# skovaka/UNCALLED

Measured on NVIDIA H100. Metric: reads/sec mapped (E. coli, 4k-sample reads) at 1/2/4/8 H100 vs CPU ref, higher is better.
Workload: dtype f32/f64 events, u32 FM index

## Files before the change

### uncalled_b200/csrc/unc_device.cuh

```cuda
#pragma once
#include "unc_warp.cuh"

typedef uint8_t u8;
typedef uint16_t u16;
typedef uint32_t u32;
typedef int32_t i32;
typedef uint64_t u64;

#define UNC_NKMER 1024
#define UNC_KMASK 0x3FFu
#define UNC_SEED_LEN 22u
#define UNC_NGEN 24u
#define UNC_PATH_MASK 0x3FFFFFu
#define UNC_PATH_TAIL 0x200000u
#define UNC_INVALID 0x80000000u
#define UNC_BLK 32u


struct DevIndex {
    const uint4 *bwt;
    const u32 *sa;
    const u32 *sa_full;
    const uint2 *kmer_range;
    const float *lv_mean, *lv_var2, *lognorm;
    const float *thresh;
    u32 primary, seq_len;
    u32 L2[5];
    u32 start_bits;
    const uint4 *occ2;
    const struct K2V2Tab *kt;
};

#define K2V2_MAX_MERGED 64u
struct alignas(16) K2V2Tab {
    u16 kslot[UNC_NKMER];
    u16 gkmer[UNC_NKMER];
    u16 gmeta[UNC_NKMER];
    u16 mk[K2V2_MAX_MERGED];
    u8 ksub[UNC_NKMER];
};

UNC_DEV u32 unc_L2(const DevIndex &ix, u32 c) {
    return c == 0 ? ix.L2[0] : c == 1 ? ix.L2[1] : c == 2 ? ix.L2[2] : c == 3 ? ix.L2[3] : ix.L2[4];
}

struct DevParams {
    u32 max_rep_copy, max_paths, max_consec_stay, max_events, min_rep_len;
    float max_stay_frac, min_seed_prob;
    u32 min_map_len;
    float min_mean_conf, min_top_conf;
    float threshold1, threshold2, peak_height, min_mean, max_mean;
    float bp_per_sec, sample_rate;
    float tgt_mean, tgt_stdv;
};

struct DevReadDesc {
    u64 offset;
    u32 n_samples, dtype;
    float cal_range, cal_offset, cal_digit;
    u32 pad;
};

struct DevRec {
    i32 mapped, fwd, rid, status;
    u32 n_events, events_used, matches, n_clusters;
// ... 598 lines not shown
            blk = de.z; cnt = de.w;
            mm.ren_start = 0; mm.evt_en = 0; mm.ref_st = 0; mm.ren_end = 0; mm.evt_st = 0; mm.total_len = 0;
            if ((u32) lane < cnt) mm = trk_load(t, blk, (u32) lane);
        }
        Clu a;
        a.ren_start = w_shfl(mm.ren_start, (int) mpos); a.evt_en = w_shfl(mm.evt_en, (int) mpos); a.ref_st = w_shfl(mm.ref_st, (int) mpos);
        a.ren_end = w_shfl(mm.ren_end, (int) mpos); a.evt_st = w_shfl(mm.evt_st, (int) mpos); a.total_len = w_shfl(mm.total_len, (int) mpos);
        u32 prev_len = a.total_len;
        clu_update(a, ns);
        if (a.total_len != prev_len) {
            t.len_sum = f_add(t.len_sum, (float) (a.total_len - prev_len));
            lens_replace(t, prev_len, a.total_len);
            if (a.total_len >= p.min_map_len && a.total_len > t.max_map.total_len) t.max_map = a;
        }
        bool in_place = false;
        if (mpos > 0) {
            const u32 ps = w_shfl(mm.ren_start, (int) mpos - 1), pe = w_shfl(mm.evt_en, (int) mpos - 1);
            in_place = clu_less(ps, pe, a.ren_start, a.evt_en);
        } else in_place = md == 0;
        if (in_place) {
            w_sync();
            if (lane == 0) {
                trk_store(t, blk, mpos, a);
                if (mpos == 0) t.dir[md] = make_uint4(a.ren_start, a.evt_en, blk, cnt);
            }
            w_sync();
        } else {
            trk_erase(t, md, mpos);
            trk_insert_unique(t, a);
        }
    } else {
        lens_insert(t, ns.total_len);
        t.len_sum = f_add(t.len_sum, (float) ns.total_len);
        if (ns.total_len >= p.min_map_len && ns.total_len > t.max_map.total_len) t.max_map = ns;
        trk_insert_unique(t, ns, have_lb ? &lb : nullptr);
    }
    PT_TRK(t, 2)
}

UNC_DEV bool trk_get_final(const Tracker &t, const DevParams &p) {
    if (t.max_map.total_len < p.min_map_len || t.n_lens < 2) return false;
    float mean_len = f_div(t.len_sum, (float) t.n_live);
    float second_len = (float) t.top2;
    float sl = (float) t.max_map.total_len;
    return (p.min_mean_conf > 0 && f_div(sl, mean_len) >= p.min_mean_conf) ||
           (p.min_top_conf > 0 && f_div(sl, second_len) >= p.min_top_conf);
}

#define K2_CH_SLOTS 160u
#define K2_V2_DYN_BYTES (16u + K2_MAXSEG * (K2_CH_SLOTS * 8u + K2_CH_SLOTS))
#ifndef K2_MAXSEG
#define K2_MAXSEG 16u
#endif
#define K2_DYN_PER_CHUNK 8u
#define K2_SMEM_BYTES(maxp) (sizeof(K2Shared) + 16 + (size_t) (((maxp) + 31) / 32) * K2_DYN_PER_CHUNK + 32 + K2_V2_DYN_BYTES)
struct K2Tables {
    uint2 kmer_range[UNC_NKMER];
    float thresh[64];
};
struct K2V2 {
    K2V2Tab t;
    u32 kcnt[UNC_NKMER];
    u32 koff[UNC_NKMER];
    u32 kagg[UNC_NKMER];
    u32 fresh_cand[32], fresh_mask[32], fresh_before[32];
    u32 grab;
    u16 mfirst[K2V2_MAX_MERGED];
#if defined(UNC_PHASE_TIMING) && !defined(UNC_EMUL)
    u32 pt_dur[4][K2_MAXSEG];
#endif
};
struct K2Shared {
    K2Tables tb;
    float probs[UNC_NKMER];
    u32 flags[32];
    u32 flags_prev[32];
    u32 sort_hist[256 * K2_MAXSEG];
    uint4 trk_dir[1024];
    u32 *bcnt, *ecnt;
    K2V2 v2;
    unsigned char *v2_stage;
    u32 bc[8];
    u32 n_rows[2];
    u32 verdict[2];
    u32 wk_overflow;
    u32 wl_cnt;
    u32 cnt_blocks, cnt_steps;
    u32 tot_children[2], tot_sources[2];
    DevWork work;
};

#include "unc_pdqsort.cuh"
#ifdef UNC_EMUL
static unsigned long g_emu_tie_stats[2];
#endif
UNC_DEV void write_source(uint4 *rec, uint2 *hist_e, u32 idx, u32 st, u32 en, u32 kmer, float prob) {
    rec[(size_t) idx * 2] = make_uint4(st, en, kmer | (1u << 16), 1u);
    rec[(size_t) idx * 2 + 1] = make_uint4(f2u(prob), f2u(prob), 0u, 0u);
    hist_e[idx] = make_uint2(f2u(prob), 0xFFFFFFFFu);
}

UNC_DEV u32 unc_event_to_bp(u32 evt_i, bool last, float mean_event_len, float bp_per_samp) {
    float v = f_add(f_mul(f_mul((float) evt_i, mean_event_len), bp_per_samp), (float) (last ? 4 : 0));
    return f_to_u32_x86(v);
}

UNC_DEV void unc_k2_cta_setup(const DevIndex &ix, const DevParams &p, K2Shared *sh) {
    const u32 n_slots = (p.max_paths + 31u) >> 5;
    if (c_tid() == 0) {
        char *base = (char *) ((((size_t) (sh + 1)) + 15) & ~(size_t) 15);
        sh->bcnt = (u32 *) base; base += (size_t) n_slots * 4;
        sh->ecnt = (u32 *) base; base += (size_t) n_slots * 4;
        sh->v2_stage = (unsigned char *) ((((size_t) base) + 15) & ~(size_t) 15);
    }
    c_sync();
    for (u32 k = (u32) c_tid(); k < UNC_NKMER; k += (u32) c_nthreads()) {
        sh->tb.kmer_range[k] = ix.kmer_range[k];
    }
    for (u32 k = (u32) c_tid(); k < 64; k += (u32) c_nthreads()) sh->tb.thresh[k] = ix.thresh[k];
    for (u32 k = (u32) c_tid(); k < (u32) (sizeof(K2V2Tab) / 4); k += (u32) c_nthreads()) ((u32 *) &sh->v2.t)[k] = ((const u32 *) ix.kt)[k];
    c_sync();
}

UNC_DEV void unc_k2_write_record(const DevIndex &ix, const DevParams &p, const DevBatch &B, K2Shared *sh, u32 r,
                                 const Tracker &trk, u32 verdict, u32 final_event, u64 n_seeds) {
    const float mel = B.mean_event_len[r];
    const float bp_per_samp = f_div(p.bp_per_sec, p.sample_rate);
    DevRec o;
    o.mapped = 0; o.fwd = 0; o.rid = -1; o.status = verdict == 2u ? -7 : 0;
    o.n_events = B.n_events[r]; o.events_used = final_event; o.matches = 0; o.n_clusters = trk.n_live;
    o.rd_len = f_to_u64(f_mul((float) (u64) B.reads[r].n_samples, bp_per_samp));
    o.rd_st = o.rd_en = o.rf_st = o.rf_en = o.rf_len = 0;
    if (verdict == 1u) {
        const Clu &sc = trk.max_map;
        bool fwd = sc.ref_st < ix.seq_len / 2u;
        u64 sa_st = fwd ? (u64) sc.ref_st : (u64) ix.seq_len - ((u64) sc.ren_end + 4u);
        o.rd_st = unc_event_to_bp(sc.evt_st - UNC_SEED_LEN, false, mel, bp_per_samp);
        o.rd_en = unc_event_to_bp(sc.evt_en, true, mel, bp_per_samp);
        o.rd_len = unc_event_to_bp(final_event, true, mel, bp_per_samp);
        int rid = -1;
        if ((long long) sa_st < (long long) B.l_pac) {
            int left = 0, mid = 0, right = (int) B.n_seqs;
            while (left < right) {
                mid = (left + right) >> 1;
                if (sa_st >= B.seq_offsets[mid]) {
                    if (mid == (int) B.n_seqs - 1) break;
                    if (sa_st < B.seq_offsets[mid + 1]) break;
                    left = mid + 1;
                } else right = mid;
            }
            rid = mid;
        }
        u64 rf_st = 0, rf_len = 0;
        if (rid >= 0) { rf_st = sa_st - B.seq_offsets[rid]; rf_len = B.seq_lens[rid]; }
        o.mapped = 1; o.fwd = fwd ? 1 : 0; o.rid = rid;
        o.rf_st = rf_st; o.rf_len = rf_len;
        o.rf_en = rf_st + ((u64) sc.ren_end - (u64) sc.ref_st + 5u);
        o.matches = (sc.total_len + 4u) & 0xFFFFu;
    }
    o.n_children = ((u64) sh->tot_children[1] << 32) | sh->tot_children[0];
    o.n_sources = ((u64) sh->tot_sources[1] << 32) | sh->tot_sources[0];
    o.n_seeds = n_seeds;
    o.n_occ_blocks = sh->cnt_blocks; o.n_sa_steps = sh->cnt_steps;
    B.out[r] = o;
}

#if defined(UNC_PHASE_TIMING) && !defined(UNC_EMUL)
UNC_DEV long long pt_clock() { long long v; asm volatile("mov.u64 %0, %%clock64;" : "=l"(v) :: "memory"); return v; }
#define PT_DECL unsigned long long pt_acc[32]; for (int _i = 0; _i < 32; _i++) pt_acc[_i] = 0; long long pt_t = pt_clock();
#define UNC_PT_TRACE_READ 40u
#define UNC_PT_TRACE_E0 60u
#define UNC_PT_TRACE_BYTES (8u * 16u * 32u * 8u)
#define PT_TRACE(ev, i, t) if ((B).dbg && r == UNC_PT_TRACE_READ && (ev) - UNC_PT_TRACE_E0 < 8u && (c_tid() & 31) == 0) \
        (B).dbg[(size_t) (B).n_reads * 64 + ((size_t) ((ev) - UNC_PT_TRACE_E0) * 16 + (c_tid() >> 5)) * 32 + (i)] = (unsigned long long) (t);
#define PT_MARK(i) { long long _n = pt_clock(); pt_acc[i] += (unsigned long long) (_n - pt_t); pt_t = _n; PT_TRACE(event_i, i, _n) }
#define PT_FLUSH(B, r) if ((B).dbg && (wt == 0 || wt == nwt - 32u)) { for (int _i = 0; _i < (wt == 0 ? 32 : 28); _i++) (B).dbg[(size_t) (r) * 64 + (wt == 0 ? 0 : 32) + _i] = pt_acc[_i]; }
#define PT_FENCE c_sync_sub(1, (int) nwt);
#define PT_WDECL long long pt_w0 = 0;
#define PT_WB pt_w0 = pt_clock();
#define PT_WE(ph) if (lane == 0) v2->pt_dur[ph][ww] = (u32) (pt_clock() - pt_w0);
#define PT_WARR(ph) if (lane == 0) v2->pt_dur[ph][ww] = (u32) pt_clock(); w_sync(); s_atomic_max(&v2->pt_dur[ph][ww], (u32) pt_clock());
#define PT_WREL(ph) if (lane == 0 && *(volatile u32 *) &v2->grab != 0xFFFFFFFFu) { const long long _t = pt_clock(); v2->pt_dur[ph][ww] = (u32) _t; PT_TRACE(event_i, 30, _t) }
#define PT_WLAG(ph, s_last, s_first) if (wt == 0) { const u32 _now = (u32) pt_clock(); u32 _mn = 0xFFFFFFFFu, _mx = 0; for (u32 _w = 0; _w < nwk; _w++) { \
        const u32 _d = _now - *(volatile u32 *) &v2->pt_dur[ph][_w]; _mn = _d < _mn ? _d : _mn; _mx = _d > _mx ? _d : _mx; } pt_acc[s_last] += _mn; pt_acc[s_first] += _mx; }
#define PT_WTRK(ph, s) if (wt == 0) pt_acc[s] += (u32) pt_clock() - *(volatile u32 *) &v2->pt_dur[ph][K2_MAXSEG - 2 + (event_i & 1u)];
#define PT_WR(ph, s_max, s_mean) if (wt == 0) { u32 _mx = 0, _sm = 0; for (u32 _w = 0; _w < nwk; _w++) { const u32 _d = *(volatile u32 *) &v2->pt_dur[ph][_w]; \
        _mx = _d > _mx ? _d : _mx; _sm += _d; } pt_acc[s_max] += _mx; pt_acc[s_mean] += _sm / nwk; }
#else
#define PT_DECL
#define PT_MARK(i)
#define PT_FLUSH(B, r)
#define PT_FENCE
#define PT_WDECL
#define PT_WB
#define PT_WE(ph)
#define PT_WARR(ph)
#define PT_WLAG(ph, s_last, s_first)
#define PT_WTRK(ph, s)
#define PT_WREL(ph)
#define PT_WR(ph, s_max, s_mean)
#endif

template <bool STREAM>
UNC_DEV void unc_k2_tracker(const DevIndex &ix, const DevParams &p, const DevBatch &B, const DevWork &W,
                            K2Shared *sh, u32 r, u32 n_first, u32 n_limit) {
    const int lane = w_lane();
    Tracker trk;
    trk.blocks = W.clu; trk.dir_glob = W.dir; trk.max_blocks = W.max_blocks;
    trk.dir = sh->trk_dir; trk.dir_cap = (u32) (sizeof(sh->trk_dir) / sizeof(uint4));
    trk_reset(trk);
    DevMapState *ms = nullptr;
    if (STREAM) {
        ms = B.mstate + B.chan[r];
        if (ms->started) {
            trk.nb = ms->t_nb; trk.n_alloc = ms->t_n_alloc; trk.n_live = ms->t_n_live; trk.n_lens = ms->t_n_lens;
            trk.top1 = ms->t_top1; trk.top2 = ms->t_top2; trk.overflow = ms->t_overflow; trk.len_sum = ms->t_len_sum;
            trk.max_map.ren_start = ms->t_max_map[0]; trk.max_map.evt_en = ms->t_max_map[1]; trk.max_map.ref_st = ms->t_max_map[2];
            trk.max_map.ren_end = ms->t_max_map[3]; trk.max_map.evt_st = ms->t_max_map[4]; trk.max_map.total_len = ms->t_max_map[5];
            if (trk.dir != trk.dir_glob) {
                if (trk.nb <= trk.dir_cap) { for (u32 j = (u32) lane; j < trk.nb; j += 32u) trk.dir[j] = trk.dir_glob[j]; w_sync(); }
                else trk.dir = trk.dir_glob;
            }
        }
    }
    u32 verdict = 0, i = n_first, final_event = n_limit;
    u64 n_seeds = 0;
#if defined(UNC_PHASE_TIMING) && !defined(UNC_EMUL)
    trk.pt[0] = trk.pt[1] = trk.pt[2] = 0;
#endif
    for (;;) {
#if defined(UNC_PHASE_TIMING) && !defined(UNC_EMUL)
        if (lane == 0) *(volatile u32 *) &sh->v2.pt_dur[3][K2_MAXSEG - 2 + (i & 1u)] = (u32) pt_clock();
        PT_TRACE(i, 0, pt_clock())
#endif
        c_sync();
        if (i == n_limit) break;
        if (verdict) { c_sync(); break; }
        const uint2 *rl = W.rlist + (size_t) (i & 1u) * W.rl_cap;
#if defined(UNC_PHASE_TIMING) && !defined(UNC_EMUL)
        const long long trk_t0 = pt_clock();
        PT_TRACE(i, 1, trk_t0)
#endif
        const u32 n = *(volatile u32 *) &sh->n_rows[i & 1u];
#if defined(UNC_PHASE_TIMING) && !defined(UNC_EMUL)
        PT_TRACE(i, 2, pt_clock())
        PT_TRACE(i, 4, n)
#endif
        for (u32 j0 = 0; j0 < n; j0 += 32u) {
            uint2 mine = make_uint2(0, 0);
            if (j0 + (u32) lane < n) mine = rl[j0 + (u32) lane];
            const u32 nj = n - j0 < 32u ? n - j0 : 32u;
            for (u32 j = 0; j < nj; j++) {
                const u32 ex = w_shfl(mine.x, (int) j), ey = w_shfl(mine.y, (int) j);
// ... 109 lines not shown
```

### uncalled_b200/csrc/unc_k2v2.cuh

```cuda
#pragma once

#define K2V2_STAGE_BYTES (K2_CH_SLOTS * 8u + K2_CH_SLOTS)


UNC_DEV void unc_occ2_build_block(const uint4 *bwt, u32 j, uint4 *out) {
    const uint4 *p = bwt + ((size_t) (j >> 1) << 2);
    const uint4 b0 = p[0], b1 = p[1];
    uint4 cnt = make_uint4(b0.x, b0.z, b1.x, b1.z);
    const uint4 lo = p[2], hi = p[3];
    if (j & 1u) {
        const u32 w[4] = {lo.x, lo.y, lo.z, lo.w};
        for (int i = 0; i < 4; i++) {
            const u32 h = w[i] >> 1, m = 0x55555555u;
            const u32 c3 = (u32) d_popc(h & w[i] & m), c2 = (u32) d_popc(h & ~w[i] & m), c1 = (u32) d_popc(~h & w[i] & m);
            cnt.x += 16u - c1 - c2 - c3; cnt.y += c1; cnt.z += c2; cnt.w += c3;
        }
    }
    out[(size_t) j * 2] = cnt;
    out[(size_t) j * 2 + 1] = (j & 1u) ? hi : lo;
}

UNC_DEV void unc_occ2_all(const uint4 cnt, const uint4 sym, u32 p, u32 o[4]) {
    u32 c1 = 0, c2 = 0, c3 = 0;
#pragma unroll
// ... 114 lines not shown
    if (use_carry) mx = mx > carry_mx ? mx : carry_mx;
    *mx_last = w_shfl(mx, 31);
    r.begin_v = a && first && prob_ok && kr.x <= cur.x - 1u;
    r.as = mx + 1u;
    r.ae = has_next ? nx - 1u : kr.y;
    r.after_v = a && !r.dup && prob_ok && r.as <= r.ae;
    r.seed = a && !r.dup && (cur.w & 1u);
    r.m_b = w_ballot(r.begin_v); r.m_a = w_ballot(r.after_v); r.m_seed = w_ballot(r.seed);
    return r;
}

#define K2V2_V_DUP 1u
#define K2V2_V_BEGIN 2u
#define K2V2_V_AFTER 4u
#define K2V2_V_SEED 8u
UNC_DEV uint4 k2v2_verdict(u32 as, u32 ae, u32 before, u32 flags, u32 kmer, u32 slot) {
    return make_uint4(as, ae, before, flags | (kmer << 4) | (slot << 14));
}
UNC_DEV u32 k2v2_flags(const K2V2Walk &w) {
    return (w.dup ? K2V2_V_DUP : 0u) | (w.begin_v ? K2V2_V_BEGIN : 0u) | (w.after_v ? K2V2_V_AFTER : 0u) | (w.seed ? K2V2_V_SEED : 0u);
}

struct K2V2Pack {
    bool a;
    u32 bl;
    u32 start, pos, n;
};
UNC_DEV K2V2Pack k2v2_next_pack(u32 cnt, u32 P, u32 *remaining) {
    const int lane = w_lane();
    const int s = d_ffs(*remaining) - 1;
    const u32 Ps = w_shfl(P, s);
    const bool fits = ((*remaining >> lane) & 1u) && (P + cnt - Ps <= 32u);
    const u32 in_pack = w_ballot(fits);
    *remaining &= ~in_pack;
    const int e = 31 - d_clz(in_pack);
    const u32 T = w_shfl(P + cnt, e) - Ps;
    K2V2Pack k;
    k.a = (u32) lane < T;
    k.bl = (u32) s; k.start = 0;
    u32 m = in_pack;
    while (m) {
        const int b = d_ffs(m) - 1;
        m &= m - 1;
        const u32 sb = w_shfl(P, b) - Ps;
        if ((u32) lane >= sb) { k.bl = (u32) b; k.start = sb; }
    }
    k.pos = (u32) lane - k.start;
    k.n = w_shfl(cnt, (int) k.bl);
    return k;
}
UNC_DEV u32 k2v2_segmask(u32 start, u32 n) { return (n >= 32u ? 0xFFFFFFFFu : ((1u << n) - 1u)) << start; }

UNC_DEV u32 k2v2_slot(u32 rank) { return ((rank & 31u) << 5) | (rank >> 5); }

UNC_DEV uint2 *k2v2_stage(K2Shared *sh, u32 ww) {
    const u32 off = (u32) (sh->v2_stage - (unsigned char *) sh) + ww * K2V2_STAGE_BYTES;
    return (uint2 *) ((unsigned char *) sh + off);
}

UNC_DEV void k2v2_add64(u32 *w, u32 v) {
    const u64 s = (((u64) w[1] << 32) | w[0]) + v;
    w[0] = (u32) s; w[1] = (u32) (s >> 32);
}

UNC_DEV u32 k2v2_grab(u32 *counter) {
    u32 g = 0;
    if (w_lane() == 0) g = s_atomic_add(counter, 1u);
    return w_shfl(g, 0);
}

UNC_DEV void k2v2_sort_small(uint4 *keys, u32 n, uint4 *sst) {
    const int lane = w_lane();
    const bool a = (u32) lane < n;
    uint4 k = make_uint4(0, 0, 0, 0);
    if (a) k = keys[lane];
    u32 rnk = 0;
    const u32 kf = k2v2_fkey(k.z), kr_ = k.w >> 14;
    for (u32 j = 0; j < n; j++) {
        const u32 jx = w_shfl(k.x, (int) j), jy = w_shfl(k.y, (int) j), jf = w_shfl(kf, (int) j), jr = w_shfl(kr_, (int) j);
        if (k2v2_less_pre(jx, jy, jf, jr, k.x, k.y, kf, kr_)) rnk++;
    }
    if (a) sst[rnk] = k;
    w_sync();
    if (a) keys[lane] = sst[lane];
    w_sync();
}

UNC_DEV u32 k2v2_walk_merged(K2Shared *sh, const uint4 *keys, uint4 *verd, u32 n, u32 moff, u32 slot, float source_prob,
                             uint4 *sst) {
    K2V2 *v2 = &sh->v2;
    const u32 lane = (u32) w_lane();
    u32 nsrc = 0, nseed = 0, prev_sub = 0xFFFFFFFFu, un_st = 1, un_en = 0;
  for (u32 g0 = 0; g0 < n; g0 += 32u) {
    const u32 cnt = n - g0 < 32u ? n - g0 : 32u;
    if (lane < cnt) sst[lane] = keys[g0 + lane];
    if (lane == 0 && g0 + cnt < n) sst[32] = keys[g0 + cnt];
    w_sync();
    if (lane == 0)
    for (u32 j = 0; j < cnt; j++) {
        const u32 i = g0 + j;
        const uint4 cur = sst[j];
        const u32 sub = (cur.w >> 6) & 0xFFu, kmer = v2->t.mk[moff + sub];
        const uint2 kr = sh->tb.kmer_range[kmer];
        const bool ok = sh->probs[kmer] >= source_prob;
        const u32 before = nsrc | (nseed << 16);
        u32 fl = 0, src_st = 0, src_en = 0;
// ... 91 lines not shown
    const u32 lt = w_lanemask_lt();
    PT_DECL
    PT_WDECL

    for (; event_i < n_limit; event_i++) {
        PT_MARK(9)
        const float event = f_add(f_mul(B.scale[r], B.events[(size_t) r * B.ev_stride + (event_i - n_first)]), B.shift[r]);
        PT_MARK(7)

        if (FLAGS && wt < 32u) sh->flags_prev[wt] = sh->flags[wt];
        for (u32 k = wt; k < UNC_NKMER; k += nwt) {
            sh->probs[k] = unc_match_prob(event, d_ldg(ix.lv_mean + k), d_ldg(ix.lv_var2 + k), d_ldg(ix.lognorm + k));
            v2->kcnt[k] = 0; v2->kagg[k] = 0;
        }
        for (u32 j = ww; j < 32; j += nwk) {
            const u32 k = j * 32 + (u32) lane;
            const float pk = unc_match_prob(event, d_ldg(ix.lv_mean + k), d_ldg(ix.lv_var2 + k), d_ldg(ix.lognorm + k));
            const uint2 kr = tb->kmer_range[k];
            const u32 m = w_ballot(pk >= source_prob && kr.x <= kr.y);
            if (lane == 0) v2->fresh_cand[j] = m;
        }
        if (wt == 0) v2->grab = 0;
        if (EXACT && wt == 0) sh->bc[5] = 0;
        if (wt < K2V2_MAX_MERGED) v2->mfirst[wt] = 0xFFFFu;
        PT_MARK(0)
        c_sync_sub(1, (int) nwt);
        PT_FENCE
        PT_MARK(16)


        const u32 nch_prev = (prev_size + 31u) >> 5;
        {
            const uint4 *prev = W.paths + (size_t) gen * gen_recs * 2;
            uint4 *next = W.paths + (size_t) (gen ^ 1u) * gen_recs * 2, *cks = W.cks;
            uint2 *hist_e = W.hist + (size_t) (event_i % UNC_NGEN) * gen_recs;
            const u32 *oprev = W.order + (size_t) gen * maxp;
            uint2 *stage_r = k2v2_stage(sh, ww);
            u8 *stage_m = (u8 *) (stage_r + K2_CH_SLOTS);
            u32 oi_n = UNC_INVALID, oi_nn = UNC_INVALID; uint4 q0_n = make_uint4(0, 0, 0, 0); uint2 q1_n = make_uint2(0, 0);
            if (ww < nch_prev) {
                const u32 pi = ww * 32u + (u32) lane;
                if (pi < prev_size) oi_n = oprev[pi];
                if (!(oi_n & UNC_INVALID)) { const uint4 *pr = prev + (size_t) oi_n * 2; q0_n = pr[0]; q1_n = *(const uint2 *) (pr + 1); }
            }
            if (ww + nwk < nch_prev) {
                const u32 pi = (ww + nwk) * 32u + (u32) lane;
                if (pi < prev_size) oi_nn = oprev[pi];
                if (!(oi_nn & UNC_INVALID)) d_prefetch(prev + (size_t) oi_nn * 2);
            }
            for (u32 c = ww; c < nch_prev; c += nwk) {
                const u32 oi = oi_n;
                const uint4 q0 = q0_n; const uint2 q1 = q1_n;
                const bool valid = !(oi & UNC_INVALID);
                oi_n = oi_nn;
                if (c + nwk < nch_prev && !(oi_n & UNC_INVALID)) {
                    const uint4 *pr = prev + (size_t) oi_n * 2;
                    q0_n = pr[0]; q1_n = *(const uint2 *) (pr + 1);
                }
                oi_nn = UNC_INVALID;
                if (c + 2u * nwk < nch_prev) {
                    const u32 pi = (c + 2u * nwk) * 32u + (u32) lane;
                    if (pi < prev_size) oi_nn = oprev[pi];
                    if (!(oi_nn & UNC_INVALID)) d_prefetch(prev + (size_t) oi_nn * 2);
                }
                const u32 st = q0.x, en = q0.y, kmer = q0.z & UNC_KMASK, plen = (q0.z >> 16) & 0xFFu, stays = (q0.z >> 24) & 0xFFu;
                const u32 moves = q0.w & UNC_PATH_MASK, sa_checked = q0.w >> 31;
                u32 want = 0, cmask = 0;
                if (valid) {
                    const float thr = tb->thresh[32 + d_clz(en - st + 1u)];
                    if (stays < p.max_consec_stay && sh->probs[kmer] >= thr) cmask = 1u;
#pragma unroll
                    for (u32 b = 0; b < 4; b++)
                        if (!(sh->probs[((kmer << 2) & UNC_KMASK) | b] < thr)) want |= 1u << b;
                }
                if (cmask) stage_r[(u32) lane * 5u] = make_uint2(st, en);
                if (want) {
                    const u32 k0 = st - 1u, l0 = en;
                    const u32 kk = k0 - (k0 >= ix.primary), ll = l0 - (l0 >= ix.primary);
                    const bool l_is_end = (l0 == ix.seq_len);
                    const uint4 *bk = ix.occ2 + ((size_t) (kk >> 6) << 1);
                    const uint4 kc = d_ldg(bk), ks = d_ldg(bk + 1);
                    uint4 lc = kc, ls = ks;
                    if (!l_is_end && (ll >> 6) != (kk >> 6)) {
                        const uint4 *bl = ix.occ2 + ((size_t) (ll >> 6) << 1);
                        lc = d_ldg(bl); ls = d_ldg(bl + 1);
                    }
                    pend_blocks += 1u + ((!l_is_end && (ll >> 7) != (kk >> 7)) ? 1u : 0u);
                    u32 ok[4], ol[4];
                    unc_occ2_all(kc, ks, kk & 63u, ok);
                    unc_occ2_all(lc, ls, ll & 63u, ol);
                    if (l_is_end) { ol[0] = ix.L2[1] - ix.L2[0]; ol[1] = ix.L2[2] - ix.L2[1]; ol[2] = ix.L2[3] - ix.L2[2]; ol[3] = ix.L2[4] - ix.L2[3]; }
#pragma unroll
                    for (u32 b = 0; b < 4; b++) {
                        const u32 nsb = ix.L2[b] + ok[b] + 1u, neb = ix.L2[b] + ol[b];
                        if (((want >> b) & 1u) && nsb <= neb) { cmask |= 2u << b; stage_r[(u32) lane * 5u + 1u + b] = make_uint2(nsb, neb); }
                    }
                }
                const u32 cc = (u32) d_popc(cmask);
                u32 total;
                const u32 off = w_exscan(cc, &total);
                bool ended = false;
                const u32 mc = (u32) d_popc(moves);
                if (valid && cc == 0 && !sa_checked) {
                    const u32 len = en - st + 1u;
                    ended = plen == UNC_SEED_LEN && u2f(q1.x) >= p.min_seed_prob &&
                            ((len == 1 && (moves & 1u) && (float) ((plen - mc) & 0xFFu) <= f_mul(p.max_stay_frac, 22.0f)) ||
                             (len <= p.max_rep_copy && mc >= p.min_rep_len));
                }
                const u32 m_ended = w_ballot(ended);
                if (ended) W.elist[(size_t) c * 32 + (u32) d_popc(m_ended & lt)] = make_uint4(st, en, mc, off);
                if (lane == 0) { sh->bcnt[c] = total; sh->ecnt[c] = (u32) d_popc(m_ended); }
                {
                    u32 pos = off;
#pragma unroll
                    for (u32 j = 0; j < 5; j++)
                        if ((cmask >> j) & 1u) { stage_m[pos] = (u8) ((u32) lane | (j << 5)); pos++; }
                }
                w_sync();
                for (u32 t0 = 0; t0 < total; t0 += 32u) {
                    const u32 t = t0 + (u32) lane;
                    const bool act = t < total;
                    u32 m = 0; uint2 rg = make_uint2(0, 0);
                    if (act) { m = stage_m[t]; rg = stage_r[(m & 31u) * 5u + (m >> 5)]; }
                    const int L = (int) (m & 31u);
                    const u32 j = m >> 5;
                    const u32 pz = w_shfl(q0.z, L), pw = w_shfl(q0.w, L), pC = w_shfl(q1.y, L), poi = w_shfl(oi, L);
                    if (act) {
                        const u32 pk = pz & UNC_KMASK, ppl = (pz >> 16) & 0xFFu, pst = (pz >> 24) & 0xFFu;
                        const u32 ckm = j == 0 ? pk : (((pk << 2) & UNC_KMASK) | (j - 1u));
                        const float pb = sh->probs[ckm];
                        const u32 move = j > 0 ? 1u : 0u;
                        const u32 nlen = ppl + (ppl < UNC_SEED_LEN ? 1u : 0u);
                        u32 nmoves = (((pw & UNC_PATH_MASK) << 1) | move) & UNC_PATH_MASK;
                        const u32 nstays = move ? 0u : pst + 1u;
                        const float newC = f_add(u2f(pC), pb);
                        const u32 ci = c * K2_CH_SLOTS + t;
                        float sp = 0.0f;
                        bool seedable = false;
                        if (ppl == UNC_SEED_LEN) {
                            nmoves |= UNC_PATH_TAIL;
                            W.wlist[s_atomic_add(&sh->wl_cnt, 1u)] = make_uint4(ci, poi, f2u(newC), nmoves);
                        } else {
                            sp = f_div(newC, (float) nlen);
                            const u32 cmc = (u32) d_popc(nmoves);
                            seedable = nlen == UNC_SEED_LEN && sp >= p.min_seed_prob && rg.x == rg.y && (nmoves & 1u) &&
                                       (float) ((nlen - cmc) & 0xFFu) <= f_mul(p.max_stay_frac, 22.0f);
                        }
                        const u32 spb = f2u(sp);
                        next[(size_t) ci * 2] = make_uint4(rg.x, rg.y, ckm | (nlen << 16) | (nstays << 24), nmoves | (pw & 0x80000000u));
                        next[(size_t) ci * 2 + 1] = make_uint4(spb, f2u(newC), 0u, 0u);
                        hist_e[ci] = make_uint2(f2u(newC), poi);
                        cks[ci] = make_uint4(rg.x, rg.y, spb, ckm | (seedable ? 1u << 10 : 0u) | ((u32) d_popc(nmoves) << 11));
                        s_atomic_add(&v2->kcnt[v2->t.kslot[ckm]], 1u);
                    }
                }
                if (c + nwk < nch_prev && !(oi_n & UNC_INVALID)) {
                    const u32 k0n = q0_n.x - 1u;
                    d_prefetch(ix.occ2 + ((size_t) ((k0n - (k0n >= ix.primary)) >> 6) << 1));
                }
                w_sync();
            }
        }
        PT_MARK(1)
        c_sync_sub(1, (int) nwt);
        PT_FENCE
        PT_MARK(17)
        if (ww == 0) {
            {
                const u32 per = (nch_prev + 31u) >> 5, c_lo = (u32) lane * per, c_hi = c_lo + per < nch_prev ? c_lo + per : nch_prev;
                u32 sum = 0;
#pragma unroll 1
                for (u32 c = c_lo; c < c_hi; c++) sum += sh->bcnt[c];
                u32 tot, run = w_exscan(sum, &tot);
#pragma unroll 1
                for (u32 c = c_lo; c < c_hi; c++) { const u32 v = sh->bcnt[c]; sh->bcnt[c] = run; run += v; }
                if (lane == 0) sh->bc[2] = tot;
            }
            w_sync();
            uint2 *rlist = W.rlist + (size_t) (event_i & 1u) * W.rl_cap;
            u32 rows = 0;
            for (u32 i0 = 0; i0 < nch_prev; i0 += 32) {
                u32 ec = i0 + (u32) lane < nch_prev ? sh->ecnt[i0 + lane] : 0u;
                u32 m = w_ballot(ec != 0);
                while (m) {
                    int l = d_ffs(m) - 1;
                    m &= m - 1;
                    u32 c = i0 + (u32) l, n = w_shfl(ec, l), base = sh->bcnt[c];
                    for (u32 j = 0; j < n; j++) {
                        uint4 e = W.elist[(size_t) c * 32 + j];
                        if (base + e.w < maxp) {
                            u32 len = e.y - e.x + 1u;
                            if (rows + len <= W.rl_cap) {
                                for (u32 i = (u32) lane; i < len; i += 32) rlist[rows + i] = make_uint2(e.x + i, e.z | 0x100u);
                            } else sh->wk_overflow = 1;
                            rows += len;
                        }
                    }
                }
            }
            if (lane == 0) sh->bc[3] = rows;
        }
        if (ww == nwk - 1u) {
            k2v2_bucket_offsets(v2);
        }
        if (ww != 0 || nwk == 1) {
            const u32 bt = nwk == 1 ? wt : wt - 32u, nbt = nwk == 1 ? nwt : nwt - 32u;
            const u32 nwl = *(volatile u32 *) &sh->wl_cnt;
            uint4 *next = W.paths + (size_t) (gen ^ 1u) * gen_recs * 2, *cks = W.cks;
            const uint2 *hist = W.hist;
            const u32 recs = (u32) gen_recs, s_e = event_i % UNC_NGEN;
            for (u32 i = bt; i < nwl; i += nbt) {
                uint4 w = W.wlist[i];
                u32 idx = w.y, s = s_e;
#pragma unroll 1
                for (u32 j = 0; j < 21u; j++) {
                    s = s ? s - 1u : UNC_NGEN - 1u;
                    idx = hist[s * recs + idx].y;
                }
                s = s ? s - 1u : UNC_NGEN - 1u;
                float oldC = u2f(hist[s * recs + idx].x);
                float sp = f_div(f_sub(u2f(w.z), oldC), 22.0f);
                uint4 key = cks[w.x];
                u32 cmc = (u32) d_popc(w.w);
                bool seedable = sp >= p.min_seed_prob && key.x == key.y && (w.w & 1u) &&
                                (float) ((UNC_SEED_LEN - cmc) & 0xFFu) <= f_mul(p.max_stay_frac, 22.0f);
                key.z = f2u(sp);
                if (seedable) key.w |= 1u << 10;
                cks[w.x] = key;
                next[(size_t) w.x * 2 + 1].x = f2u(sp);
            }
        }
        PT_MARK(10)
        c_sync_sub(1, (int) nwt);
        PT_FENCE
        PT_MARK(26)
        if (wt == 0) sh->wl_cnt = 0;
        const u32 nc_total = nch_prev ? sh->bc[2] : 0u;
        const u32 nc = nc_total < maxp ? nc_total : maxp;
        if (nc_total > maxp) {
            for (u32 c = ww; c < nch_prev; c += nwk) {
                const u32 base = sh->bcnt[c], end = c + 1 < nch_prev ? sh->bcnt[c + 1] : nc_total;
                if (end <= nc) continue;
                for (u32 i = (base < nc ? nc - base : 0u) + (u32) lane; base + i < end; i += 32)
                    s_atomic_add(&v2->kagg[v2->t.kslot[W.cks[(size_t) c * K2_CH_SLOTS + i].w & UNC_KMASK]], 1u);
            }
            c_sync_sub(1, (int) nwt);
            if (ww == 0) {
                const u32 l = (u32) lane;
#pragma unroll 1
                for (u32 j = 0; j < 32; j++) {
                    const u32 sl = j * 32u + l;
                    const u32 nxt = j < 31u ? v2->koff[sl + 32u] : (l < 31u ? v2->koff[l + 1u] : nc_total);
                    v2->kcnt[sl] = nxt - v2->koff[sl] - v2->kagg[sl];
                    v2->kagg[sl] = 0;
                }
                w_sync();
                k2v2_bucket_offsets(v2);
            }
            c_sync_sub(1, (int) nwt);
        }
        PT_MARK(12)
        u32 n_rows = sh->bc[3];
        if (n_rows > W.rl_cap) n_rows = W.rl_cap;
        const u32 n_ended_rows = n_rows;

        if (nc > 0) {
          {
            uint4 *ckA = W.ckey;
            const uint4 *cks = W.cks;
            uint4 kpre = make_uint4(0, 0, 0, 0);
            if (ww < nch_prev) {
                const u32 b0 = sh->bcnt[ww], e0 = ww + 1 < nch_prev ? sh->bcnt[ww + 1] : nc_total;
                if (b0 + (u32) lane < e0 && b0 + (u32) lane < nc) kpre = cks[(size_t) ww * K2_CH_SLOTS + (u32) lane];
            }
            for (u32 c = ww; c < nch_prev; c += nwk) {
                const u32 base = sh->bcnt[c];
                if (base >= nc) break;
                const u32 end = c + 1 < nch_prev ? sh->bcnt[c + 1] : nc_total;
                const uint4 kcur = kpre;
                if (c + nwk < nch_prev) {
                    const u32 bn = sh->bcnt[c + nwk], en = c + nwk + 1 < nch_prev ? sh->bcnt[c + nwk + 1] : nc_total;
                    if (bn + (u32) lane < en && bn + (u32) lane < nc) kpre = cks[(size_t) (c + nwk) * K2_CH_SLOTS + (u32) lane];
                }
                for (u32 i = (u32) lane; base + i < end && base + i < nc; i += 32) {
                    const u32 ci = c * K2_CH_SLOTS + i;
                    uint4 key = i < 32u ? kcur : cks[ci];
                    const u32 km = key.w & UNC_KMASK;
                    const u32 bk = v2->t.kslot[km];
                    key.w = ((key.w >> 10) & 0x3Fu) | ((u32) v2->t.ksub[km] << 6) | (ci << 14);
                    ckA[s_atomic_add(&v2->kcnt[bk], 1u)] = key;
                }
            }
          }
            PT_MARK(2)
            c_sync_sub(1, (int) nwt);
            PT_FENCE
            PT_MARK(18)
            PT_WB

            uint4 *ckA = W.ckey, *ckB = W.ckey + maxp;
            uint2 *stage_r = k2v2_stage(sh, ww);
            u32 *whist = sh->sort_hist + (size_t) ww * 256u;
          for (bool recount = false;; recount = true) {
            const bool sort = !(EXACT && recount);
            for (;;) {
                const u32 gi = k2v2_grab(&v2->grab);
                if (gi >= 96u) break;
                const u32 grp = gi & 31u;
                const u32 sl = (u32) lane * 32u + grp;
                const u32 bo = v2->koff[sl], bn = v2->kcnt[sl] - bo;
                const u32 meta = v2->t.gmeta[grp * 32u + (u32) lane];
                if (gi < 64u) {
                    const bool huge_sweep = gi < 32u;
                    u32 todo_m = huge_sweep ? w_ballot(meta != 0 && bn > 0) : 0u;
                    while (todo_m) {
                        const int l = d_ffs(todo_m) - 1;
                        todo_m &= todo_m - 1;
// ... 48 lines not shown
                    const u32 cnt = (bn > 0 && bn <= 32u && meta == 0) ? bn : 0u;
                    u32 tot;
                    const u32 P = w_exscan(cnt, &tot);
                    u32 remaining = w_ballot(cnt != 0);
                    while (remaining) {
                        const K2V2Pack pk = k2v2_next_pack(cnt, P, &remaining);
                        const u32 addr = w_shfl(bo, (int) pk.bl) + pk.pos;
                        uint4 k = make_uint4(0, 0, 0, 0);
                        if (pk.a) k = ckA[addr];
                        u32 rnk = pk.pos;
                        if (sort) {
                            const u32 maxn = w_max(pk.a ? pk.n : 0u);
                            rnk = 0;
                            const u32 kf = k2v2_fkey(k.z), kri = k.w >> 14;
                            for (u32 q = 0; q < maxn; q++) {
                                const int src = (int) ((pk.start + q) & 31u);
                                const u32 jx = w_shfl(k.x, src), jy = w_shfl(k.y, src), jf = w_shfl(kf, src), jr = w_shfl(kri, src);
                                if (pk.a && q < pk.n && k2v2_less_pre(jx, jy, jf, jr, k.x, k.y, kf, kri)) rnk++;
                            }
                        }
                        uint4 *sst = (uint4 *) stage_r;
                        if (pk.a) sst[pk.start + rnk] = k;
                        w_sync();
                        uint4 cur = make_uint4(0, 0, 0, 0);
                        if (pk.a) { cur = sst[lane]; ckA[addr] = cur; }
                        w_sync();
                        const u32 nx = w_shfl_down(cur.x, 1), ny = w_shfl_down(cur.y, 1);
                        const u32 kmer = v2->t.gkmer[grp * 32u + pk.bl];
                        const uint2 kr = tb->kmer_range[kmer];
                        const bool prob_ok = sh->probs[kmer] >= source_prob;
                        u32 mxo;
                        const K2V2Walk wk = k2v2_walk(cur, nx, ny, pk.a, pk.a && pk.pos + 1u < pk.n, pk.pos == 0, pk.pos == 0, false, 0u,
                                                      prob_ok, kr, &mxo);
                        const u32 sm = k2v2_segmask(pk.start, pk.n);
                        if (pk.a) {
                            const u32 src_b = (u32) d_popc(wk.m_b & lt & sm) + (u32) d_popc(wk.m_a & lt & sm), seed_b = (u32) d_popc(wk.m_seed & lt & sm);
                            ckB[addr] = k2v2_verdict(wk.as, wk.ae, src_b | (seed_b << 16), k2v2_flags(wk), kmer, pk.bl * 32u + grp);
                        }
                        if (pk.a && pk.pos == 0)
                            v2->kagg[pk.bl * 32u + grp] = ((u32) d_popc(wk.m_b & sm) + (u32) d_popc(wk.m_a & sm)) | ((u32) d_popc(wk.m_seed & sm) << 16);
                    }
                }
            }
            PT_WE(1)
            PT_MARK(3)
            c_sync_sub(1, (int) nwt);
            if (!EXACT || recount || !k2v2_exact_order(sh, W, nc, maxp, wt, nwt)) break;
          }
            PT_FENCE
            PT_MARK(19)
            PT_WR(1, 15, 20)
        }

        if (ww == 0) {
            u32 sum = 0;
#pragma unroll 1
            for (u32 j = 0; j < 32; j++) sum += v2->kagg[j * 32u + (u32) lane];
            u32 ts, tq;
            const u32 es = w_exscan(sum & 0xFFFFu, &ts), eq = w_exscan(sum >> 16, &tq);
            u32 run = es | (eq << 16);
#pragma unroll 1
            for (u32 j = 0; j < 32; j++) {
                const u32 sl = j * 32u + (u32) lane, v = v2->kagg[sl];
                v2->kagg[sl] = run;
                if (nc > 0 && v2->kcnt[sl] != v2->koff[sl]) {
                    const u32 meta = v2->t.gmeta[(u32) lane * 32u + j];
                    if (meta == 0) {
                        const u32 kmer = v2->t.gkmer[(u32) lane * 32u + j];
                        if (sh->probs[kmer] >= source_prob && nc + (run & 0xFFFFu) < maxp) s_atomic_or(&sh->flags[kmer >> 5], 1u << (kmer & 31u));
                    } else {
                        for (u32 m = 0; m < (meta & 0xFFu); m++) {
                            const u32 f = v2->mfirst[(meta >> 8) + m], kmer = v2->t.mk[(meta >> 8) + m];
                            if (f != 0xFFFFu && sh->probs[kmer] >= source_prob && nc + (run & 0xFFFFu) + f < maxp)
                                s_atomic_or(&sh->flags[kmer >> 5], 1u << (kmer & 31u));
                        }
                    }
                }
                run = ((run & 0xFFFFu) + (v & 0xFFFFu)) | (((run >> 16) + (v >> 16)) << 16);
            }
            w_sync();
            const u32 tot_src = ts;
            const u32 ns_added = nc + tot_src > maxp ? maxp - nc : tot_src;
            const u32 nn0 = nc + ns_added;
            const u32 my_mask = v2->fresh_cand[lane] & ~sh->flags[lane];
            u32 tot_add;
            const u32 my_pre = w_exscan((u32) d_popc(my_mask), &tot_add);
            v2->fresh_mask[lane] = my_mask;
            v2->fresh_before[lane] = nn0 + my_pre;
            if (lane == 0) {
                sh->bc[1] = nn0 + tot_add < maxp ? nn0 + tot_add : maxp;
                sh->bc[6] = tq;
            }
        }
        if (ww != 0 || nwk == 1) {
            const u32 bt = nwk == 1 ? wt : wt - 32u, nbt = nwk == 1 ? nwt : nwt - 32u;
            uint2 *rlist = W.rlist + (size_t) (event_i & 1u) * W.rl_cap;
            for (u32 i = bt; i < n_ended_rows; i += nbt) {
                uint2 e = rlist[i];
                e.x = ix.seq_len - unc_sa_lookup(ix, e.x, &pend_steps, &pend_blocks);
                rlist[i] = e;
            }
        }
        PT_MARK(11)
        c_sync_sub(1, (int) nwt);
        PT_FENCE
        PT_MARK(27)
        PT_WB
        const u32 n_child_seeds = nc > 0 ? sh->bc[6] : 0u;
        n_rows = n_ended_rows + n_child_seeds;
        if (n_rows > W.rl_cap) n_rows = W.rl_cap;

        if (nc > 0) {
            const uint4 *ckA = W.ckey, *verd = W.ckey + maxp;
            uint4 *next = W.paths + (size_t) (gen ^ 1u) * gen_recs * 2;
            uint2 *hist_e = W.hist + (size_t) (event_i % UNC_NGEN) * gen_recs;
            u32 *onext = W.order + (size_t) (gen ^ 1u) * maxp;
            uint2 *rlist = W.rlist + (size_t) (event_i & 1u) * W.rl_cap;
            for (u32 i = wt; i < nc; i += nwt) {
                const uint4 cur = ckA[i], v = verd[i];
                const u32 rec = cur.w >> 14;
                onext[i] = rec | ((v.w & K2V2_V_DUP) ? UNC_INVALID : 0u);
                if (!(v.w & (K2V2_V_BEGIN | K2V2_V_AFTER | K2V2_V_SEED))) continue;
                const u32 kmer = (v.w >> 4) & 1023u, pre = v2->kagg[v.w >> 14];
                if (v.w & (K2V2_V_BEGIN | K2V2_V_AFTER)) {
                    const float pkm = sh->probs[kmer];
                    u32 sidx = (pre & 0xFFFFu) + (v.z & 0xFFFFu);
                    if (v.w & K2V2_V_BEGIN) {
                        if (nc + sidx < maxp) {
                            write_source(next, hist_e, S0 + nc + sidx, tb->kmer_range[kmer].x, cur.x - 1u, kmer, pkm);
                            onext[nc + sidx] = S0 + nc + sidx;
                        }
                        sidx++;
                    }
                    if ((v.w & K2V2_V_AFTER) && nc + sidx < maxp) {
                        write_source(next, hist_e, S0 + nc + sidx, v.x, v.y, kmer, pkm);
                        onext[nc + sidx] = S0 + nc + sidx;
                    }
                }
                if (v.w & K2V2_V_SEED) {
                    d_atomic_or(&((u32 *) (next + (size_t) rec * 2))[3], 0x80000000u);
                    const u32 ri = n_ended_rows + (pre >> 16) + (v.z >> 16);
                    if (ri < W.rl_cap)
                        rlist[ri] = make_uint2(ix.seq_len - unc_sa_lookup(ix, cur.x, &pend_steps, &pend_blocks), (cur.w >> 1) & 0x1Fu);
                    else sh->wk_overflow = 1;
                }
            }
        }
        PT_WE(2)
        uint4 *next = W.paths + (size_t) (gen ^ 1u) * gen_recs * 2;
        uint2 *hist_e = W.hist + (size_t) (event_i % UNC_NGEN) * gen_recs;
        u32 *onext = W.order + (size_t) (gen ^ 1u) * maxp;
        for (u32 j = ww; j < 32; j += nwk) {
            const u32 before = v2->fresh_before[j];
            if (before >= maxp) continue;
            const u32 k = j * 32 + (u32) lane;
            const u32 fw = sh->flags[j];
            u32 m_add = v2->fresh_mask[j];
            const u32 room = maxp - before;
            u32 visited = 0xFFFFFFFFu;
// ... 47 lines not shown
```

Baseline: 5498.

## Add checkpoint jump ring for seed history walk and parallelize row scans across warps

Adds a jump-pointer ring, written every UNC_CKPT events and carried in each path record, so the 21-step history walk for full-length seeds can skip 12 steps at once. It also precomputes per-chunk ended-row counts so that writing the row list is spread across all warps instead of done by warp 0, and splits the k-mer aggregate prefix scan across warps using an extra barrier. The goal is to shorten serial per-event phases. In exchange it adds global memory for the ring, extra shared memory, and extra barriers, and it shrinks the history ring to 23 generations.

```diff
diff --git a/uncalled_b200/csrc/unc_device.cuh b/uncalled_b200/csrc/unc_device.cuh
--- a/uncalled_b200/csrc/unc_device.cuh
+++ b/uncalled_b200/csrc/unc_device.cuh
@@ -10,7 +10,8 @@
 #define UNC_NKMER 1024
 #define UNC_KMASK 0x3FFu
 #define UNC_SEED_LEN 22u
-#define UNC_NGEN 24u
+#define UNC_NGEN 23u
+#define UNC_CKPT 12u
 #define UNC_PATH_MASK 0x3FFFFFu
 #define UNC_PATH_TAIL 0x200000u
 #define UNC_INVALID 0x80000000u
@@ -715,7 +716,7 @@
 #ifndef K2_MAXSEG
 #define K2_MAXSEG 16u
 #endif
-#define K2_DYN_PER_CHUNK 8u
+#define K2_DYN_PER_CHUNK 12u
 #define K2_SMEM_BYTES(maxp) (sizeof(K2Shared) + 16 + (size_t) (((maxp) + 31) / 32) * K2_DYN_PER_CHUNK + 32 + K2_V2_DYN_BYTES)
 struct K2Tables {
     uint2 kmer_range[UNC_NKMER];
@@ -730,7 +731,7 @@
     u32 grab;
     u16 mfirst[K2V2_MAX_MERGED];
 #if defined(UNC_PHASE_TIMING) && !defined(UNC_EMUL)
-    u32 pt_dur[4][K2_MAXSEG];
+    u32 pt_dur[6][K2_MAXSEG];
 #endif
 };
 struct K2Shared {
@@ -741,6 +742,7 @@
     u32 sort_hist[256 * K2_MAXSEG];
     uint4 trk_dir[1024];
     u32 *bcnt, *ecnt;
+    u32 *erow;
     K2V2 v2;
     unsigned char *v2_stage;
     u32 bc[8];
@@ -759,7 +761,7 @@
 #endif
 UNC_DEV void write_source(uint4 *rec, uint2 *hist_e, u32 idx, u32 st, u32 en, u32 kmer, float prob) {
     rec[(size_t) idx * 2] = make_uint4(st, en, kmer | (1u << 16), 1u);
-    rec[(size_t) idx * 2 + 1] = make_uint4(f2u(prob), f2u(prob), 0u, 0u);
+    rec[(size_t) idx * 2 + 1] = make_uint4(f2u(prob), f2u(prob), 0xFFFFFFFFu, 0u);
     hist_e[idx] = make_uint2(f2u(prob), 0xFFFFFFFFu);
 }
 
@@ -774,6 +776,7 @@
         char *base = (char *) ((((size_t) (sh + 1)) + 15) & ~(size_t) 15);
         sh->bcnt = (u32 *) base; base += (size_t) n_slots * 4;
         sh->ecnt = (u32 *) base; base += (size_t) n_slots * 4;
+        sh->erow = (u32 *) base; base += (size_t) n_slots * 4;
         sh->v2_stage = (unsigned char *) ((((size_t) base) + 15) & ~(size_t) 15);
     }
     c_sync();
@@ -849,6 +852,8 @@
 #define PT_WTRK(ph, s) if (wt == 0) pt_acc[s] += (u32) pt_clock() - *(volatile u32 *) &v2->pt_dur[ph][K2_MAXSEG - 2 + (event_i & 1u)];
 #define PT_WR(ph, s_max, s_mean) if (wt == 0) { u32 _mx = 0, _sm = 0; for (u32 _w = 0; _w < nwk; _w++) { const u32 _d = *(volatile u32 *) &v2->pt_dur[ph][_w]; \
         _mx = _d > _mx ? _d : _mx; _sm += _d; } pt_acc[s_max] += _mx; pt_acc[s_mean] += _sm / nwk; }
+#define PT_WR_LAST(ph, s_max, s_mean) if (wt == nwt - 32u) { u32 _mx = 0, _sm = 0; for (u32 _w = 0; _w < nwk; _w++) { const u32 _d = *(volatile u32 *) &v2->pt_dur[ph][_w]; \
+        _mx = _d > _mx ? _d : _mx; _sm += _d; } pt_acc[s_max] += _mx; pt_acc[s_mean] += _sm / nwk; }
 #else
 #define PT_DECL
 #define PT_MARK(i)
@@ -862,6 +867,7 @@
 #define PT_WTRK(ph, s)
 #define PT_WREL(ph)
 #define PT_WR(ph, s_max, s_mean)
+#define PT_WR_LAST(ph, s_max, s_mean)
 #endif
 
 template <bool STREAM>
diff --git a/uncalled_b200/csrc/unc_k2v2.cuh b/uncalled_b200/csrc/unc_k2v2.cuh
--- a/uncalled_b200/csrc/unc_k2v2.cuh
+++ b/uncalled_b200/csrc/unc_k2v2.cuh
@@ -190,6 +190,8 @@
 UNC_DEV u32 k2v2_segmask(u32 start, u32 n) { return (n >= 32u ? 0xFFFFFFFFu : ((1u << n) - 1u)) << start; }
 
 UNC_DEV u32 k2v2_slot(u32 rank) { return ((rank & 31u) << 5) | (rank >> 5); }
+
+UNC_DEV u32 *k2v2_jump_ring(const DevWork &W, size_t gen_recs) { return (u32 *) (W.hist + (size_t) UNC_NGEN * gen_recs); }
 
 UNC_DEV uint2 *k2v2_stage(K2Shared *sh, u32 ww) {
     const u32 off = (u32) (sh->v2_stage - (unsigned char *) sh) + ww * K2V2_STAGE_BYTES;
@@ -387,6 +389,7 @@
                 const u32 oi = oi_n;
                 const uint4 q0 = q0_n; const uint2 q1 = q1_n;
                 const bool valid = !(oi & UNC_INVALID);
+                const u32 pj = valid ? prev[(size_t) oi * 2 + 1].z : 0u;
                 oi_n = oi_nn;
                 if (c + nwk < nch_prev && !(oi_n & UNC_INVALID)) {
                     const uint4 *pr = prev + (size_t) oi_n * 2;
@@ -444,7 +447,9 @@
                 }
                 const u32 m_ended = w_ballot(ended);
                 if (ended) W.elist[(size_t) c * 32 + (u32) d_popc(m_ended & lt)] = make_uint4(st, en, mc, off);
-                if (lane == 0) { sh->bcnt[c] = total; sh->ecnt[c] = (u32) d_popc(m_ended); }
+                u32 erows = 0;
+                if (m_ended) w_exscan(ended ? en - st + 1u : 0u, &erows);
+                if (lane == 0) { sh->bcnt[c] = total; sh->ecnt[c] = (u32) d_popc(m_ended); sh->erow[c] = erows; }
                 {
                     u32 pos = off;
 #pragma unroll
@@ -459,7 +464,7 @@
                     if (act) { m = stage_m[t]; rg = stage_r[(m & 31u) * 5u + (m >> 5)]; }
                     const int L = (int) (m & 31u);
                     const u32 j = m >> 5;
-                    const u32 pz = w_shfl(q0.z, L), pw = w_shfl(q0.w, L), pC = w_shfl(q1.y, L), poi = w_shfl(oi, L);
+                    const u32 pz = w_shfl(q0.z, L), pw = w_shfl(q0.w, L), pC = w_shfl(q1.y, L), poi = w_shfl(oi, L), pJ = w_shfl(pj, L);
                     if (act) {
                         const u32 pk = pz & UNC_KMASK, ppl = (pz >> 16) & 0xFFu, pst = (pz >> 24) & 0xFFu;
                         const u32 ckm = j == 0 ? pk : (((pk << 2) & UNC_KMASK) | (j - 1u));
@@ -470,11 +475,12 @@
                         const u32 nstays = move ? 0u : pst + 1u;
                         const float newC = f_add(u2f(pC), pb);
                         const u32 ci = c * K2_CH_SLOTS + t;
+                        const u32 cj = (event_i - 1u) % UNC_CKPT == 0u ? poi : pJ;
                         float sp = 0.0f;
                         bool seedable = false;
                         if (ppl == UNC_SEED_LEN) {
                             nmoves |= UNC_PATH_TAIL;
-                            W.wlist[s_atomic_add(&sh->wl_cnt, 1u)] = make_uint4(ci, poi, f2u(newC), nmoves);
+                            W.wlist[s_atomic_add(&sh->wl_cnt, 1u)] = make_uint4(ci, cj, f2u(newC), nmoves);
                         } else {
                             sp = f_div(newC, (float) nlen);
                             const u32 cmc = (u32) d_popc(nmoves);
@@ -483,8 +489,9 @@
                         }
                         const u32 spb = f2u(sp);
                         next[(size_t) ci * 2] = make_uint4(rg.x, rg.y, ckm | (nlen << 16) | (nstays << 24), nmoves | (pw & 0x80000000u));
-                        next[(size_t) ci * 2 + 1] = make_uint4(spb, f2u(newC), 0u, 0u);
+                        next[(size_t) ci * 2 + 1] = make_uint4(spb, f2u(newC), cj, 0u);
                         hist_e[ci] = make_uint2(f2u(newC), poi);
+                        if (event_i % UNC_CKPT == 0u) k2v2_jump_ring(W, gen_recs)[(size_t) ((event_i / UNC_CKPT) & 1u) * gen_recs + ci] = cj;
                         cks[ci] = make_uint4(rg.x, rg.y, spb, ckm | (seedable ? 1u << 10 : 0u) | ((u32) d_popc(nmoves) << 11));
                         s_atomic_add(&v2->kcnt[v2->t.kslot[ckm]], 1u);
                     }
@@ -500,40 +507,31 @@
         c_sync_sub(1, (int) nwt);
         PT_FENCE
         PT_MARK(17)
+        PT_WB
         if (ww == 0) {
-            {
-                const u32 per = (nch_prev + 31u) >> 5, c_lo = (u32) lane * per, c_hi = c_lo + per < nch_prev ? c_lo + per : nch_prev;
-                u32 sum = 0;
+            const u32 per = (nch_prev + 31u) >> 5, c_lo = (u32) lane * per, c_hi = c_lo + per < nch_prev ? c_lo + per : nch_prev;
+            u32 sum = 0;
 #pragma unroll 1
-                for (u32 c = c_lo; c < c_hi; c++) sum += sh->bcnt[c];
-                u32 tot, run = w_exscan(sum, &tot);
+            for (u32 c = c_lo; c < c_hi; c++) sum += sh->bcnt[c];
+            u32 tot, run = w_exscan(sum, &tot), rsum = 0;
 #pragma unroll 1
-                for (u32 c = c_lo; c < c_hi; c++) { const u32 v = sh->bcnt[c]; sh->bcnt[c] = run; run += v; }
-                if (lane == 0) sh->bc[2] = tot;
-            }
-            w_sync();
-            uint2 *rlist = W.rlist + (size_t) (event_i & 1u) * W.rl_cap;
-            u32 rows = 0;
-            for (u32 i0 = 0; i0 < nch_prev; i0 += 32) {
-                u32 ec = i0 + (u32) lane < nch_prev ? sh->ecnt[i0 + lane] : 0u;
-                u32 m = w_ballot(ec != 0);
-                while (m) {
-                    int l = d_ffs(m) - 1;
-                    m &= m - 1;
-                    u32 c = i0 + (u32) l, n = w_shfl(ec, l), base = sh->bcnt[c];
-                    for (u32 j = 0; j < n; j++) {
-                        uint4 e = W.elist[(size_t) c * 32 + j];
-                        if (base + e.w < maxp) {
-                            u32 len = e.y - e.x + 1u;
-                            if (rows + len <= W.rl_cap) {
-                                for (u32 i = (u32) lane; i < len; i += 32) rlist[rows + i] = make_uint2(e.x + i, e.z | 0x100u);
-                            } else sh->wk_overflow = 1;
-                            rows += len;
-                        }
+            for (u32 c = c_lo; c < c_hi; c++) {
+                const u32 v = sh->bcnt[c];
+                u32 rw = sh->erow[c];
+                if (run + v >= maxp) {
+                    rw = 0;
+                    for (u32 j = 0; run < maxp && j < sh->ecnt[c]; j++) {
+                        const uint4 e = W.elist[(size_t) c * 32 + j];
+                        if (run + e.w < maxp) rw += e.y - e.x + 1u;
                     }
                 }
-            }
-            if (lane == 0) sh->bc[3] = rows;
+                sh->bcnt[c] = run; sh->erow[c] = rw;
+                run += v; rsum += rw;
+            }
+            u32 rtot, rrun = w_exscan(rsum, &rtot);
+#pragma unroll 1
+            for (u32 c = c_lo; c < c_hi; c++) { const u32 v = sh->erow[c]; sh->erow[c] = rrun; rrun += v; }
+            if (lane == 0) { sh->bc[2] = tot; sh->bc[3] = rtot; }
         }
         if (ww == nwk - 1u) {
             k2v2_bucket_offsets(v2);
@@ -543,16 +541,23 @@
             const u32 nwl = *(volatile u32 *) &sh->wl_cnt;
             uint4 *next = W.paths + (size_t) (gen ^ 1u) * gen_recs * 2, *cks = W.cks;
             const uint2 *hist = W.hist;
-            const u32 recs = (u32) gen_recs, s_e = event_i % UNC_NGEN;
+            const u32 *jump = k2v2_jump_ring(W, gen_recs);
+            const u32 recs = (u32) gen_recs, d = (event_i - 1u) % UNC_CKPT;
+            const u32 s_j = (event_i + UNC_NGEN - 1u - d) % UNC_NGEN;
+            const u32 j_j = ((event_i - 1u - d) / UNC_CKPT) & 1u;
             for (u32 i = bt; i < nwl; i += nbt) {
                 uint4 w = W.wlist[i];
-                u32 idx = w.y, s = s_e;
+                u32 idx = w.y, s = s_j, left = 21u - d;
+                if (left >= UNC_CKPT) {
+                    idx = jump[j_j * recs + idx];
+                    left -= UNC_CKPT;
+                    s = s >= UNC_CKPT ? s - UNC_CKPT : s + UNC_NGEN - UNC_CKPT;
+                }
 #pragma unroll 1
-                for (u32 j = 0; j < 21u; j++) {
+                for (; left > 0; left--) {
+                    idx = hist[s * recs + idx].y;
                     s = s ? s - 1u : UNC_NGEN - 1u;
-                    idx = hist[s * recs + idx].y;
-                }
-                s = s ? s - 1u : UNC_NGEN - 1u;
+                }
                 float oldC = u2f(hist[s * recs + idx].x);
                 float sp = f_div(f_sub(u2f(w.z), oldC), 22.0f);
                 uint4 key = cks[w.x];
@@ -565,10 +570,12 @@
                 next[(size_t) w.x * 2 + 1].x = f2u(sp);
             }
         }
+        PT_WE(4)
         PT_MARK(10)
         c_sync_sub(1, (int) nwt);
         PT_FENCE
         PT_MARK(26)
+        PT_WR_LAST(4, 13, 14)
         if (wt == 0) sh->wl_cnt = 0;
         const u32 nc_total = nch_prev ? sh->bc[2] : 0u;
         const u32 nc = nc_total < maxp ? nc_total : maxp;
@@ -598,6 +605,24 @@
         u32 n_rows = sh->bc[3];
         if (n_rows > W.rl_cap) n_rows = W.rl_cap;
         const u32 n_ended_rows = n_rows;
+        {
+            uint2 *rlist = W.rlist + (size_t) (event_i & 1u) * W.rl_cap;
+            for (u32 c0 = ww; c0 < nch_prev; c0 += 32u * nwk) {
+                const u32 c = c0 + (u32) lane * nwk;
+                u32 n = 0, base = 0, row = 0;
+                if (c < nch_prev) { n = sh->ecnt[c]; base = sh->bcnt[c]; row = sh->erow[c]; }
+                for (u32 j = 0; j < n && base < maxp; j++) {
+                    const uint4 e = W.elist[(size_t) c * 32 + j];
+                    if (base + e.w >= maxp) break;
+                    const u32 len = e.y - e.x + 1u;
+                    if (row + len <= W.rl_cap) {
+                        for (u32 i = 0; i < len; i++) rlist[row + i] = make_uint2(e.x + i, e.z | 0x100u);
+                    } else sh->wk_overflow = 1;
+                    row += len;
+                }
+            }
+            if (nc == 0) c_sync_sub(1, (int) nwt);
+        }
 
         if (nc > 0) {
           {
@@ -752,15 +777,23 @@
             PT_WR(1, 15, 20)
         }
 
-        if (ww == 0) {
+        PT_WB
+        u32 ts, tq;
+        {
+            u32 *bsum = sh->sort_hist;
+            const u32 per = (32u + nwk - 1u) / nwk, j_lo = ww * per < 32u ? ww * per : 32u, j_hi = j_lo + per < 32u ? j_lo + per : 32u;
             u32 sum = 0;
 #pragma unroll 1
-            for (u32 j = 0; j < 32; j++) sum += v2->kagg[j * 32u + (u32) lane];
-            u32 ts, tq;
-            const u32 es = w_exscan(sum & 0xFFFFu, &ts), eq = w_exscan(sum >> 16, &tq);
-            u32 run = es | (eq << 16);
+            for (u32 j = j_lo; j < j_hi; j++) sum += v2->kagg[j * 32u + (u32) lane];
+            bsum[ww * 32u + (u32) lane] = sum;
+            c_sync_sub(1, (int) nwt);
+            u32 gt = 0, before = 0;
 #pragma unroll 1
-            for (u32 j = 0; j < 32; j++) {
+            for (u32 w = 0; w < nwk; w++) { const u32 b = bsum[w * 32u + (u32) lane]; gt += b; if (w < ww) before += b; }
+            const u32 es = w_exscan(gt & 0xFFFFu, &ts), eq = w_exscan(gt >> 16, &tq);
+            u32 run = (es + (before & 0xFFFFu)) | ((eq + (before >> 16)) << 16);
+#pragma unroll 1
+            for (u32 j = j_lo; j < j_hi; j++) {
                 const u32 sl = j * 32u + (u32) lane, v = v2->kagg[sl];
                 v2->kagg[sl] = run;
                 if (nc > 0 && v2->kcnt[sl] != v2->koff[sl]) {
@@ -778,7 +811,9 @@
                 }
                 run = ((run & 0xFFFFu) + (v & 0xFFFFu)) | (((run >> 16) + (v >> 16)) << 16);
             }
-            w_sync();
+        }
+        c_sync_sub(1, (int) nwt);
+        if (ww == 0) {
             const u32 tot_src = ts;
             const u32 ns_added = nc + tot_src > maxp ? maxp - nc : tot_src;
             const u32 nn0 = nc + ns_added;
@@ -801,10 +836,12 @@
                 rlist[i] = e;
             }
         }
+        PT_WE(5)
         PT_MARK(11)
         c_sync_sub(1, (int) nwt);
         PT_FENCE
         PT_MARK(27)
+        PT_WR_LAST(5, 15, 20)
         PT_WB
         const u32 n_child_seeds = nc > 0 ? sh->bc[6] : 0u;
         n_rows = n_ended_rows + n_child_seeds;
```

Result: no change. 5553, median of 6 (+1.0%).
